# eminwux/kukeon

Hardware: AMD Instinct MI355X
Metric: agent_turns_per_sec (higher is better)
Workload: dtype bf16; 1 GPU; model=llama-3-8b, global_batch=64, seq_len=3584, parallelism=dp1, sessions_per_gpu_group=64, prompt_len=512, followup_len=256, decode_len=128

## Files before the change

### kukeon_amd/models/llama.py

```python
from __future__ import annotations

from dataclasses import dataclass
from typing import Optional

import torch
import torch.nn as nn
import torch.nn.functional as F

from kukeon_amd import ops
from kukeon_amd import parallel
from kukeon_amd.engine.config import ModelConfig


@dataclass
class AttnMeta:
    mode: str
    positions: torch.Tensor
    slot_mapping: torch.Tensor
    block_table: torch.Tensor
    seq_lens: torch.Tensor
    q_starts: Optional[torch.Tensor] = None
    qb_seq: Optional[torch.Tensor] = None
    qb_start: Optional[torch.Tensor] = None
    num_splits: int = 1
# ... 49 lines not shown
        import os
        weight_dtype = os.environ.get("KUKEON_WEIGHT_DTYPE") or "bf16"
    if weight_dtype not in WEIGHT_DTYPES:
        raise ValueError(f"weight_dtype must be one of {WEIGHT_DTYPES}, "
                         f"got {weight_dtype!r}")
    return weight_dtype


def _make_weight(shape, device, weight_dtype: str):
    w = _init_weight(shape, device)
    if weight_dtype == "fp8":
        return ops.quantize_weight(w.data)
    return w


class LlamaAttention(nn.Module):
    def __init__(self, cfg: ModelConfig, layer_idx: int, device,
                 weight_dtype: str = "bf16"):
        super().__init__()
        tp = parallel.tp_size()
        assert cfg.num_q_heads % tp == 0 and cfg.num_kv_heads % tp == 0, (
            "TP degree must divide q and kv head counts")
        self.layer_idx = layer_idx
        self.hq = cfg.num_q_heads // tp
        self.hk = cfg.num_kv_heads // tp
        self.d = cfg.head_dim
        self.scale = cfg.head_dim ** -0.5
        qkv_out = (self.hq + 2 * self.hk) * self.d
        self.qkv_w = _make_weight((qkv_out, cfg.hidden_size), device,
                                  weight_dtype)
        self.o_w = _make_weight((cfg.hidden_size, self.hq * self.d), device,
                                weight_dtype)

    def forward(self, x: torch.Tensor, cos_sin: torch.Tensor,
                kc: torch.Tensor, vc: torch.Tensor, meta: AttnMeta):
        qkv = ops.linear(x, self.qkv_w)
        ops.rope_kv_append(qkv, kc, vc, cos_sin, meta.positions,
                           meta.slot_mapping, self.hq, self.hk, self.d,
                           block_table=(meta.block_table
                                        if meta.mode == "decode" else None))
        out = torch.empty(x.shape[0], self.hq * self.d, dtype=x.dtype,
                          device=x.device)
        if meta.mode == "decode":
            ops.paged_attention(out, qkv, kc, vc, meta.block_table,
                                meta.seq_lens, 0, meta.num_splits, self.scale,
                                meta.tmp_out, meta.tmp_ml)
        else:
            ops.prefill_attention(out, qkv, kc, vc, meta.block_table,
                                  meta.seq_lens, meta.q_starts, meta.qb_seq,
                                  meta.qb_start, 0, self.scale)
        o = ops.linear(out, self.o_w)
        return parallel.tp_all_reduce(o)

    def forward_pre_o(self, x: torch.Tensor, cos_sin: torch.Tensor,
                      kc: torch.Tensor, vc: torch.Tensor, meta: AttnMeta):
        qkv = ops.linear(x, self.qkv_w)
        ops.rope_kv_append(qkv, kc, vc, cos_sin, meta.positions,
                           meta.slot_mapping, self.hq, self.hk, self.d,
                           block_table=(meta.block_table
                                        if meta.mode == "decode" else None))
        out = torch.empty(x.shape[0], self.hq * self.d, dtype=x.dtype,
                          device=x.device)
        if meta.mode == "decode":
            ops.paged_attention(out, qkv, kc, vc, meta.block_table,
                                meta.seq_lens, 0, meta.num_splits, self.scale,
                                meta.tmp_out, meta.tmp_ml)
        else:
            ops.prefill_attention(out, qkv, kc, vc, meta.block_table,
                                  meta.seq_lens, meta.q_starts, meta.qb_seq,
                                  meta.qb_start, 0, self.scale)
        return out


class LlamaMLP(nn.Module):
    def __init__(self, cfg: ModelConfig, device, weight_dtype: str = "bf16"):
        super().__init__()
        tp = parallel.tp_size()
        assert cfg.intermediate_size % tp == 0
        self.inter = cfg.intermediate_size // tp
        self.gate_up_w = _make_weight((2 * self.inter, cfg.hidden_size),
                                      device, weight_dtype)
        self.down_w = _make_weight((cfg.hidden_size, self.inter), device,
                                   weight_dtype)

    def forward(self, x: torch.Tensor) -> torch.Tensor:
        gu = ops.linear(x, self.gate_up_w)
        act = torch.empty(x.shape[0], self.inter, dtype=x.dtype,
                          device=x.device)
        ops.silu_mul(act, gu)
        return parallel.tp_all_reduce(ops.linear(act, self.down_w))


class LlamaLayer(nn.Module):
    def __init__(self, cfg: ModelConfig, layer_idx: int, device,
                 weight_dtype: str = "bf16"):
        super().__init__()
        self.input_norm = nn.Parameter(
            torch.ones(cfg.hidden_size, dtype=torch.bfloat16, device=device),
            requires_grad=False)
        self.post_norm = nn.Parameter(
            torch.ones(cfg.hidden_size, dtype=torch.bfloat16, device=device),
            requires_grad=False)
        self.attn = LlamaAttention(cfg, layer_idx, device, weight_dtype)
        self.mlp = LlamaMLP(cfg, device, weight_dtype)
# ... 148 lines not shown
```

### kukeon_amd/ops/__init__.py

```python
from __future__ import annotations

import torch

from . import reference

_C = None
_IMPORT_ERROR: Exception | None = None


def _load() -> None:
    global _C, _IMPORT_ERROR
    try:
        from kukeon_amd import _C as ext
    except Exception as e:
        _IMPORT_ERROR = e
    else:
        _C, _IMPORT_ERROR = ext, None


_load()


def native_available() -> bool:
    if _C is None:
# ... 17 lines not shown


def rmsnorm(out, input, weight, eps: float) -> None:
    _impl(input).rmsnorm(out, input, weight, eps)


def fused_add_rmsnorm(input, residual, weight, eps: float) -> None:
    _impl(input).fused_add_rmsnorm(input, residual, weight, eps)


def silu_mul(out, gate_up) -> None:
    _impl(gate_up).silu_mul(out, gate_up)


def rope_kv_append(qkv, k_cache, v_cache, cos_sin, positions, slot_mapping,
                   num_q_heads: int, num_kv_heads: int, head_dim: int,
                   block_table=None) -> None:
    if block_table is None:
        block_table = torch.empty(0, dtype=torch.int32, device=qkv.device)
    _impl(qkv).rope_kv_append(qkv, k_cache, v_cache, cos_sin, positions,
                              slot_mapping, num_q_heads, num_kv_heads,
                              head_dim, block_table)


def decode_advance(ids, pos, seq_lens, tokens, ring, counter) -> None:
    _impl(ids).decode_advance(ids, pos, seq_lens, tokens, ring, counter)


def paged_attention(out, q, k_cache, v_cache, block_table, seq_lens,
                    q_offset: int, num_splits: int, scale: float,
                    tmp_out, tmp_ml) -> None:
    _impl(q).paged_attention(out, q, k_cache, v_cache, block_table, seq_lens,
                             q_offset, num_splits, scale, tmp_out, tmp_ml)


def prefill_attention(out, q, k_cache, v_cache, block_table, seq_lens,
                      q_starts, qb_seq, qb_start, q_offset: int,
                      scale: float) -> None:
    _impl(q).prefill_attention(out, q, k_cache, v_cache, block_table,
                               seq_lens, q_starts, qb_seq, qb_start, q_offset,
                               scale)


def sample(tokens, logits, temps, top_k, top_p, seed, workspace) -> None:
    _impl(logits).sample(tokens, logits, temps, top_k, top_p, seed, workspace)


_SKINNY_WS = {}
_SKINNY_WS_RETIRED = []
_USE_SKINNY = __import__("os").environ.get("KUKEON_SKINNY_GEMM", "0")
_FUSE_SILU = __import__("os").environ.get("KUKEON_FUSE_SILU", "0") == "1"


def _skinny_wins(rows: int, N: int, K: int) -> bool:
    if _USE_SKINNY == "off":
        return False
    return N == K == 4096


def _skinny5_wins(rows: int, N: int, K: int) -> bool:
    if _USE_SKINNY == "off":
        return False
    return (N, K) in ((4096, 14336), (8192, 28672))


def _skinny_kind(x: torch.Tensor, w: torch.Tensor, fused: bool):
# ... 214 lines not shown
```

### kukeon_amd/ops/csrc/bindings.cpp

```cpp
#include <torch/extension.h>

namespace kukeon {
void rmsnorm(torch::Tensor out, torch::Tensor input, torch::Tensor weight,
             double eps);
void fused_add_rmsnorm(torch::Tensor input, torch::Tensor residual,
                       torch::Tensor weight, double eps);
void silu_mul(torch::Tensor out, torch::Tensor gate_up);
void rope_kv_append(torch::Tensor qkv, torch::Tensor k_cache,
                    torch::Tensor v_cache, torch::Tensor cos_sin,
                    torch::Tensor positions, torch::Tensor slot_mapping,
                    int64_t num_q_heads, int64_t num_kv_heads,
                    int64_t head_dim, torch::Tensor block_table);
void decode_advance(torch::Tensor ids, torch::Tensor pos,
                    torch::Tensor seq_lens, torch::Tensor tokens,
                    torch::Tensor ring, torch::Tensor counter);
void paged_attention(torch::Tensor out, torch::Tensor q, torch::Tensor k_cache,
                     torch::Tensor v_cache, torch::Tensor block_table,
                     torch::Tensor seq_lens, int64_t q_offset,
                     int64_t num_splits, double scale, torch::Tensor tmp_out,
                     torch::Tensor tmp_ml);
void prefill_attention(torch::Tensor out, torch::Tensor q,
                       torch::Tensor k_cache, torch::Tensor v_cache,
                       torch::Tensor block_table, torch::Tensor seq_lens,
                       torch::Tensor q_starts, torch::Tensor qb_seq,
                       torch::Tensor qb_start, int64_t q_offset, double scale);
void mfma_probe(torch::Tensor out, torch::Tensor a, torch::Tensor b);
void mfma_probe16(torch::Tensor out, torch::Tensor a, torch::Tensor b);
void mfma_probe16k(torch::Tensor out, torch::Tensor a, torch::Tensor b);
void skinny_gemm2(torch::Tensor out, torch::Tensor x, torch::Tensor w,
                  torch::Tensor ws);
void skinny_gemm5(torch::Tensor out, torch::Tensor x, torch::Tensor w,
                  torch::Tensor ws);
void skinny_gemm6(torch::Tensor out, torch::Tensor x, torch::Tensor w,
                  torch::Tensor ws);
void skinny_gemm5_silu_fused_norm(torch::Tensor normed, torch::Tensor gu,
                                  torch::Tensor w, torch::Tensor ws,
                                  torch::Tensor residual, torch::Tensor nw,
                                  double eps);
void skinny_gemm(torch::Tensor out, torch::Tensor x, torch::Tensor w,
                 torch::Tensor ws);
void glds_probe(torch::Tensor out, torch::Tensor src);
int64_t skinny_splitk(const std::string& kind, int64_t N, int64_t K);
void skinny_gemm5_fused_norm(torch::Tensor normed, torch::Tensor x,
                             torch::Tensor w, torch::Tensor ws,
                             torch::Tensor residual, torch::Tensor nw,
                             double eps);
void skinny_gemm_fused_norm(torch::Tensor normed, torch::Tensor x,
                            torch::Tensor w, torch::Tensor ws,
                            torch::Tensor residual, torch::Tensor nw,
                            double eps);
void skinny_gemm_w8(torch::Tensor out, torch::Tensor x, torch::Tensor q,
                    torch::Tensor scale, torch::Tensor ws);
void skinny_gemm_w8_fused_norm(torch::Tensor normed, torch::Tensor x,
// ... 2 lines not shown
                               torch::Tensor nw, double eps);
void quantize_fp8_rows(torch::Tensor q, torch::Tensor scale, torch::Tensor w);
void dequant_fp8_rows(torch::Tensor out, torch::Tensor q,
                      torch::Tensor scale);
void sample(torch::Tensor tokens, torch::Tensor logits, torch::Tensor temps,
            torch::Tensor top_k, torch::Tensor top_p, torch::Tensor seed,
            torch::Tensor workspace);
void moe_router_weights(torch::Tensor wdense, torch::Tensor logits,
                        long K);
void moe_dense_combine(torch::Tensor out, torch::Tensor y,
                       torch::Tensor wdense);
void moe_gather_tokens(torch::Tensor out, torch::Tensor input,
                       torch::Tensor row_map);
void moe_scatter_tokens(torch::Tensor out, torch::Tensor input,
                        torch::Tensor row_map, torch::Tensor weights,
                        int64_t top_k);
void moe_route_sort(torch::Tensor topk_w, torch::Tensor row_map,
                    torch::Tensor inv_map, torch::Tensor offsets,
                    torch::Tensor logits, long K);
void moe_grouped_gemm(torch::Tensor out, torch::Tensor a,
                      torch::Tensor a_rows, torch::Tensor w,
                      torch::Tensor offsets);
}

PYBIND11_MODULE(TORCH_EXTENSION_NAME, m) {
  m.def("rmsnorm", &kukeon::rmsnorm, "RMSNorm (bf16, gfx950)");
  m.def("fused_add_rmsnorm", &kukeon::fused_add_rmsnorm,
        "residual += input; input = rmsnorm(residual)");
  m.def("silu_mul", &kukeon::silu_mul, "out = silu(gate)*up from fused [T,2I]");
  m.def("rope_kv_append", &kukeon::rope_kv_append,
        "in-place NEOX RoPE on fused qkv + paged KV append");
  m.def("paged_attention", &kukeon::paged_attention,
        "decode paged attention (GQA, split-KV)");
  m.def("prefill_attention", &kukeon::prefill_attention,
        "varlen causal paged prefill attention (MFMA)");
  m.def("mfma_probe", &kukeon::mfma_probe,
        "32x32x16 bf16 MFMA fragment-layout probe");
  m.def("mfma_probe16", &kukeon::mfma_probe16,
        "16x16x32 bf16 MFMA fragment-layout probe");
  m.def("mfma_probe16k", &kukeon::mfma_probe16k,
        "16x16x16 (K=16) bf16 MFMA fragment-layout probe");
  m.def("skinny_gemm6", &kukeon::skinny_gemm6,
        "decode GEMM v6 (barrier-free register-x pipeline)");
  m.def("skinny_gemm5_silu_fused_norm",
        &kukeon::skinny_gemm5_silu_fused_norm,
        "silu(gate)*up + down GEMM + reduce + add + RMSNorm fused");
  m.def("skinny_gemm5", &kukeon::skinny_gemm5,
        "full-line W stream via wave-private LDS image (v5)");
  m.def("skinny_gemm2", &kukeon::skinny_gemm2,
        "G-walk hand-counted weight-streaming GEMM (v2)");
  m.def("skinny_gemm", &kukeon::skinny_gemm,
        "weight-streaming decode GEMM (M<=64)");
  m.def("skinny_splitk", &kukeon::skinny_splitk,
        "split-K factor the skinny launcher of `kind` (v1, v2, v5, v5_fused, "
        "v6, w8) uses for [N, K]; host-only",
        py::arg("kind"), py::arg("N"), py::arg("K"));
  m.def("glds_probe", &kukeon::glds_probe,
        "asm global_lds round-trip validator");
  m.def("skinny_gemm5_fused_norm", &kukeon::skinny_gemm5_fused_norm,
        "skinny5 + fused split-K reduce + residual add + RMSNorm");
  m.def("skinny_gemm_fused_norm", &kukeon::skinny_gemm_fused_norm,
        "skinny GEMM + split-K reduce + residual add + RMSNorm");
  m.def("skinny_gemm_w8", &kukeon::skinny_gemm_w8,
        "W8A16 decode GEMM: (x @ fp8(q)^T) * scale, M<=64");
  m.def("skinny_gemm_w8_fused_norm", &kukeon::skinny_gemm_w8_fused_norm,
        "W8A16 decode GEMM + split-K reduce + residual add + RMSNorm");
// ... 20 lines not shown
```

### kukeon_amd/ops/csrc/common.h

```cpp
#pragma once

#include <hip/hip_runtime.h>
#include <hip/hip_bf16.h>
#include <hip/hip_fp16.h>
#include <stdint.h>

#define WAVE 64

#define DEV_INLINE __device__ __forceinline__

DEV_INLINE float bf2f(__hip_bfloat16 x) { return __bfloat162float(x); }
DEV_INLINE __hip_bfloat16 f2bf(float x) { return __float2bfloat16(x); }

DEV_INLINE float us2f(unsigned short u) {
  unsigned int w = ((unsigned int)u) << 16;
  return __builtin_bit_cast(float, w);
}
DEV_INLINE unsigned short f2us(float f) {
  unsigned int w = __builtin_bit_cast(unsigned int, f);
  unsigned int lsb = (w >> 16) & 1u;
  w += 0x7fffu + lsb;
  return (unsigned short)(w >> 16);
}

struct bf16x8 {
  uint4 raw;
  DEV_INLINE unsigned short us(int i) const {
    const unsigned int* p = reinterpret_cast<const unsigned int*>(&raw);
    return (unsigned short)((p[i >> 1] >> ((i & 1) * 16)) & 0xffffu);
  }
  DEV_INLINE float f(int i) const { return us2f(us(i)); }
};

DEV_INLINE bf16x8 load_bf16x8(const void* p) {
  bf16x8 v;
  v.raw = *reinterpret_cast<const uint4*>(p);
  return v;
}

DEV_INLINE uint4 pack_bf16x8(const float* f) {
  uint4 r;
  unsigned int* p = reinterpret_cast<unsigned int*>(&r);
#pragma unroll
  for (int i = 0; i < 4; ++i) {
    p[i] = (unsigned int)f2us(f[2 * i]) | ((unsigned int)f2us(f[2 * i + 1]) << 16);
  }
  return r;
}

typedef __attribute__((__vector_size__(2 * sizeof(float)))) float f32x2_cvt_t;

DEV_INLINE unsigned int cvtpk_bf16(float lo, float hi) {
  __hip_bfloat162 h = __float22bfloat162_rn(float2{lo, hi});
  unsigned int r;
  __builtin_memcpy(&r, &h, 4);
  return r;
}

DEV_INLINE uint2 fp8x4_to_bf16x4(unsigned int w) {
  f32x2_cvt_t lo = __builtin_amdgcn_cvt_pk_f32_fp8(w, false);
  f32x2_cvt_t hi = __builtin_amdgcn_cvt_pk_f32_fp8(w, true);
  return uint2{cvtpk_bf16(lo[0], lo[1]), cvtpk_bf16(hi[0], hi[1])};
}

DEV_INLINE uint4 fp8x8_to_bf16x8(uint2 w) {
  const uint2 a = fp8x4_to_bf16x4(w.x);
  const uint2 b = fp8x4_to_bf16x4(w.y);
  return uint4{a.x, a.y, b.x, b.y};
}

DEV_INLINE uint2 pack_fp8x8(const float* f) {
  unsigned int w0 = __builtin_amdgcn_cvt_pk_fp8_f32(f[0], f[1], 0u, false);
  w0 = __builtin_amdgcn_cvt_pk_fp8_f32(f[2], f[3], w0, true);
  unsigned int w1 = __builtin_amdgcn_cvt_pk_fp8_f32(f[4], f[5], 0u, false);
  w1 = __builtin_amdgcn_cvt_pk_fp8_f32(f[6], f[7], w1, true);
  return uint2{w0, w1};
}

DEV_INLINE float wave_sum(float v) {
#pragma unroll
// ... 38 lines not shown
```

### kukeon_amd/ops/csrc/paged_attn.hip

```cpp
#include "attn_frag.h"
#include <torch/extension.h>
#include <c10/hip/HIPStream.h>

namespace kukeon {

template <bool FP8>
__global__ __launch_bounds__(256, FP8 ? 3 : 4) void paged_attn_kernel(
    float* __restrict__ tmp_out,
    float* __restrict__ tmp_ml,
    const unsigned short* __restrict__ q,
    const void* __restrict__ k_cache,
    const void* __restrict__ v_cache,
    const int* __restrict__ block_table,
    const int* __restrict__ seq_lens,
    long q_stride, int Hq, int Hk, int max_blocks, int S, float scale) {
  constexpr int D = 128;
  constexpr int BS = 16;
  const int b = blockIdx.x;
  const int hk = blockIdx.y;
  const int wid = threadIdx.x / WAVE;
  const int lane = threadIdx.x & (WAVE - 1);
  const int g4 = lane >> 4;
  const int rc = lane & 15;
  const int G = Hq / Hk;
  const int slot = blockIdx.z * 4 + wid;
  const int ctx = seq_lens[b];
  if (ctx <= 0 || slot >= S) return;

  __shared__ __align__(16) unsigned short vtbuf[4][2][D * BS];

  const int nblocks = (ctx + BS - 1) / BS;
  const int per_slot = (nblocks + S - 1) / S;
  const int blk_begin = slot * per_slot;
  const int blk_end = min(nblocks, blk_begin + per_slot);
  const int kv_hi = min(ctx, blk_end * BS);

  const int qh = min(rc, G - 1);
  unsigned int qf[4][4];
  {
    const unsigned short* qp =
        q + (long)b * q_stride + (long)(hk * G + qh) * D;
#pragma unroll
    for (int st = 0; st < 4; ++st) {
      const uint4 v = *reinterpret_cast<const uint4*>(qp + st * 32 + g4 * 8);
      qf[st][0] = v.x; qf[st][1] = v.y; qf[st][2] = v.z; qf[st][3] = v.w;
    }
  }

  float m = -INFINITY, l_acc = 0.f;
  f32x4_t oacc[8] = {{}, {}, {}, {}, {}, {}, {}, {}};

  const auto* kc = reinterpret_cast<const kv_elem_t<FP8>*>(k_cache);
  const auto* vc = reinterpret_cast<const kv_elem_t<FP8>*>(v_cache);

  uint4 kfr[4];
  auto kfetch = [&](int bi_f) {
    const long base =
        ((long)block_table[(long)b * max_blocks + bi_f] * Hk + hk) * BS * D;
    const long off = base + (long)rc * D + g4 * 8;
#pragma unroll
    for (int st = 0; st < 4; ++st)
      kfr[st] = load_kv8(kc + off + st * 32);
  };
  const int stg_d0 = rc * 8;
  uint4 vpre[2][2];
  auto vfetch = [&](int bi_f) {
    const long base =
        ((long)block_table[(long)b * max_blocks + bi_f] * Hk + hk) * BS * D;
#pragma unroll
    for (int pass = 0; pass < 2; ++pass) {
      const int kp = pass * 4 + g4;
      const long voff0 = base + (long)(2 * kp) * D + stg_d0;
      const long voff1 = base + (long)(2 * kp + 1) * D + stg_d0;
      vpre[pass][0] = load_kv8(vc + voff0);
      vpre[pass][1] = load_kv8(vc + voff1);
    }
  };
  auto vwrite = [&](unsigned short* vt, int kvbase) {
#pragma unroll
    for (int pass = 0; pass < 2; ++pass) {
      const int kp = pass * 4 + g4;
      uint4 r0 = vpre[pass][0];
      uint4 r1 = vpre[pass][1];
      if (kvbase + 2 * kp >= kv_hi) r0 = uint4{0, 0, 0, 0};
      if (kvbase + 2 * kp + 1 >= kv_hi) r1 = uint4{0, 0, 0, 0};
      const unsigned int* a0 = reinterpret_cast<const unsigned int*>(&r0);
      const unsigned int* a1 = reinterpret_cast<const unsigned int*>(&r1);
#pragma unroll
      for (int j = 0; j < 8; ++j) {
        const unsigned short e0 = (a0[j >> 1] >> ((j & 1) * 16)) & 0xffffu;
        const unsigned short e1 = (a1[j >> 1] >> ((j & 1) * 16)) & 0xffffu;
        const unsigned int packed = (unsigned)e0 | ((unsigned)e1 << 16);
        const int d = stg_d0 + j;
        const int byte = d * 32 + ((4 * kp) ^ ((d & 3) << 3));
        *reinterpret_cast<unsigned int*>(
            reinterpret_cast<char*>(vt) + byte) = packed;
      }
    }
  };

  if (blk_begin < blk_end) {
    kfetch(blk_begin);
    vfetch(blk_begin);
    vwrite(vtbuf[wid][blk_begin & 1], blk_begin * BS);
  }

  for (int bi = blk_begin; bi < blk_end; ++bi) {
    const int kvbase = bi * BS;
    const unsigned short* vt = vtbuf[wid][bi & 1];

    f32x4_t sacc = {};
#pragma unroll
    for (int st = 0; st < 4; ++st) {
      sacc = __builtin_amdgcn_mfma_f32_16x16x32_bf16(
          as_frag(kfr[st].x, kfr[st].y, kfr[st].z, kfr[st].w),
          as_frag(qf[st][0], qf[st][1], qf[st][2], qf[st][3]),
          sacc, 0, 0, 0);
    }
    if (bi + 1 < blk_end) kfetch(bi + 1);

    float sv[4];
    float tmax = -INFINITY;
#pragma unroll
    for (int r = 0; r < 4; ++r) {
      const bool valid = (kvbase + 4 * g4 + r) < kv_hi;
      sv[r] = valid ? sacc[r] * scale : -INFINITY;
      tmax = fmaxf(tmax, sv[r]);
    }
    tmax = fmaxf(tmax, __shfl_xor(tmax, 16, WAVE));
    tmax = fmaxf(tmax, __shfl_xor(tmax, 32, WAVE));
    const float mn = fmaxf(m, tmax);
    const float alpha = (m == -INFINITY) ? 0.f : __expf(m - mn);
    m = mn;
    float psum = 0.f;
#pragma unroll
    for (int r = 0; r < 4; ++r) {
      sv[r] = (sv[r] == -INFINITY) ? 0.f : __expf(sv[r] - mn);
      psum += sv[r];
    }
    psum += __shfl_xor(psum, 16, WAVE);
    psum += __shfl_xor(psum, 32, WAVE);
    l_acc = l_acc * alpha + psum;
#pragma unroll
    for (int dc = 0; dc < 8; ++dc)
#pragma unroll
      for (int r = 0; r < 4; ++r) oacc[dc][r] *= alpha;

    if (bi + 1 < blk_end) {
      vfetch(bi + 1);
      vwrite(vtbuf[wid][(bi + 1) & 1], (bi + 1) * BS);
    }

    const bf16x4_t pfrag = as_frag(cvtpk_bf16(sv[0], sv[1]),
                                   cvtpk_bf16(sv[2], sv[3]));
#pragma unroll
    for (int dc = 0; dc < 8; ++dc) {
      const int d = dc * 16 + rc;
      const int byte = d * 32 + ((8 * g4) ^ ((d & 3) << 3));
      const uint2 vf = *reinterpret_cast<const uint2*>(
          reinterpret_cast<const char*>(vt) + byte);
      oacc[dc] = __builtin_amdgcn_mfma_f32_16x16x16bf16_1k(
          as_frag(vf.x, vf.y), pfrag, oacc[dc], 0, 0, 0);
    }
  }

  if (rc >= G) return;
  const int head = hk * G + rc;
  float* top = tmp_out + (((long)b * Hq + head) * S + slot) * D;
#pragma unroll
  for (int dc = 0; dc < 8; ++dc) {
#pragma unroll
    for (int r = 0; r < 4; ++r) {
      top[dc * 16 + 4 * g4 + r] = oacc[dc][r];
    }
  }
  if (g4 == 0) {
    float* ml = tmp_ml + (((long)b * Hq + head) * S + slot) * 2;
    ml[0] = m;
    ml[1] = l_acc;
  }
}

template <int D>
__global__ void paged_attn_reduce_kernel(
    unsigned short* __restrict__ out, const float* __restrict__ tmp_out,
    const float* __restrict__ tmp_ml, const int* __restrict__ seq_lens,
    int Hq, int S) {
  const int b = blockIdx.x;
  const int h = blockIdx.y;
  const int d = threadIdx.x;
  if (seq_lens[b] <= 0) return;
  const float* ml = tmp_ml + (((long)b * Hq + h) * S) * 2;
  float M = -INFINITY;
  for (int s = 0; s < S; ++s) M = fmaxf(M, ml[s * 2]);
  float L = 0.f;
  for (int s = 0; s < S; ++s)
    L += (ml[s * 2] == -INFINITY ? 0.f : __expf(ml[s * 2] - M)) *
         ml[s * 2 + 1];
  const float* top = tmp_out + (((long)b * Hq + h) * S) * D;
  float acc = 0.f;
  for (int s = 0; s < S; ++s) {
    const float w = ml[s * 2] == -INFINITY ? 0.f : __expf(ml[s * 2] - M);
    acc += w * top[(long)s * D + d];
  }
  out[(long)b * Hq * D + (long)h * D + d] = f2us(L > 0.f ? acc / L : 0.f);
}

void paged_attention(torch::Tensor out, torch::Tensor q, torch::Tensor k_cache,
                     torch::Tensor v_cache, torch::Tensor block_table,
                     torch::Tensor seq_lens, int64_t q_offset,
                     int64_t num_splits, double scale, torch::Tensor tmp_out,
                     torch::Tensor tmp_ml) {
  const int B = q.size(0);
  if (B == 0) return;
  TORCH_CHECK(k_cache.dim() == 4 && k_cache.size(2) == 16 &&
                  k_cache.size(3) == 128,
              "kv caches must be [NB, Hk, 16, 128] (block size 16, "
              "head_dim 128)");
  TORCH_CHECK(v_cache.sizes() == k_cache.sizes() &&
                  v_cache.scalar_type() == k_cache.scalar_type() &&
                  k_cache.is_contiguous() && v_cache.is_contiguous(),
              "k_cache and v_cache must be contiguous and alike");
  const bool fp8 = k_cache.scalar_type() == torch::kUInt8;
  TORCH_CHECK(fp8 || k_cache.scalar_type() == torch::kBFloat16,
              "kv caches must be bf16 or uint8 (fp8 e4m3)");
  constexpr int D = 128;
  const int Hk = k_cache.size(1);
  TORCH_CHECK(out.dim() == 2 && out.size(0) == B && out.size(1) % D == 0 &&
                  out.scalar_type() == torch::kBFloat16 && out.is_contiguous(),
              "out must be contiguous bf16 [B, Hq*128]");
  const int Hq = out.size(1) / D;
  TORCH_CHECK(Hq >= Hk && Hq % Hk == 0 && Hq / Hk <= 16,
              "GQA group Hq/Hk must be an integer <= 16, got Hq=", Hq,
              " Hk=", Hk);
  TORCH_CHECK(q.scalar_type() == torch::kBFloat16 && q.dim() == 2 &&
                  q.stride(1) == 1,
              "q must be bf16 [B, >= Hq*128] with unit inner stride");
  TORCH_CHECK(q.stride(0) % 8 == 0 && q_offset % 8 == 0 && q_offset >= 0 &&
                  q_offset + (int64_t)Hq * D <= q.size(1),
              "q.stride(0) and q_offset must be multiples of 8 and the heads "
              "must fit in a q row, got stride ", q.stride(0), " offset ",
              q_offset);
  TORCH_CHECK(block_table.scalar_type() == torch::kInt32 &&
                  block_table.dim() == 2 && block_table.is_contiguous() &&
                  block_table.size(0) >= B,
              "block_table must be contiguous int32 [>= B, max_blocks]");
  TORCH_CHECK(seq_lens.scalar_type() == torch::kInt32 &&
                  seq_lens.is_contiguous() && seq_lens.numel() >= B,
              "seq_lens must be contiguous int32 [>= B]");
  TORCH_CHECK(num_splits >= 1, "num_splits must be >= 1");
  const int64_t slots = (int64_t)B * Hq * num_splits;
  TORCH_CHECK(tmp_out.scalar_type() == torch::kFloat32 &&
                  tmp_out.is_contiguous() && tmp_out.numel() >= slots * D,
              "tmp_out must be contiguous float32 with >= B*Hq*num_splits*128 "
              "elements, got ", tmp_out.numel(), " need ", slots * D);
  TORCH_CHECK(tmp_ml.scalar_type() == torch::kFloat32 &&
                  tmp_ml.is_contiguous() && tmp_ml.numel() >= slots * 2,
              "tmp_ml must be contiguous float32 with >= B*Hq*num_splits*2 "
              "elements, got ", tmp_ml.numel(), " need ", slots * 2);
  for (const auto& t : {out, k_cache, v_cache, block_table, seq_lens, tmp_out,
                        tmp_ml})
    TORCH_CHECK(t.device() == q.device() && t.is_cuda(),
                "all tensors must be on the same GPU");

  auto stream = c10::hip::getCurrentHIPStream().stream();
  const unsigned short* qp =
      reinterpret_cast<const unsigned short*>(q.data_ptr()) + q_offset;
  auto* launch = fp8 ? paged_attn_kernel<true> : paged_attn_kernel<false>;
  launch<<<dim3(B, Hk, (unsigned)((num_splits + 3) / 4)), 256, 0, stream>>>(
      tmp_out.data_ptr<float>(), tmp_ml.data_ptr<float>(), qp,
      k_cache.data_ptr(), v_cache.data_ptr(), block_table.data_ptr<int>(),
      seq_lens.data_ptr<int>(), q.stride(0), Hq, Hk,
      (int)block_table.size(1), (int)num_splits, (float)scale);
  HIP_CHECK_KERNEL();
  paged_attn_reduce_kernel<128><<<dim3(B, Hq), 128, 0, stream>>>(
      reinterpret_cast<unsigned short*>(out.data_ptr()),
      tmp_out.data_ptr<float>(), tmp_ml.data_ptr<float>(),
      seq_lens.data_ptr<int>(), Hq, (int)num_splits);
  HIP_CHECK_KERNEL();
}

}
```

### kukeon_amd/ops/csrc/rope_kv.hip

```cpp
#include "common.h"
#include <torch/extension.h>
#include <c10/hip/HIPStream.h>

namespace kukeon {

template <bool FP8>
__global__ void rope_kv_kernel(
    unsigned short* __restrict__ qkv,
    void* __restrict__ k_cache,
    void* __restrict__ v_cache,
    const float* __restrict__ cos_sin,
    const int* __restrict__ positions,
    const int* __restrict__ slot_mapping,
    const int* __restrict__ block_table,
    int max_blocks,
    int Hq, int Hk, int D, int BS) {
  const long t = blockIdx.x;
  const int yoff = blockIdx.y * blockDim.x + threadIdx.x;
  const int ystride = gridDim.y * blockDim.x;
  const int half = D / 2;
  const long row_stride = (long)(Hq + 2 * Hk) * D;
  unsigned short* row = qkv + t * row_stride;
  const int pos = positions[t];
  if (pos < 0) return;
  int slot;
  if (block_table != nullptr) {
    slot = block_table[t * (long)max_blocks + pos / BS] * BS + pos % BS;
  } else {
    slot = slot_mapping[t];
  }
  const float* cs = cos_sin + (long)pos * D;

  const int q_chunks = Hq * (D / 16);
  for (int c = yoff; c < q_chunks; c += ystride) {
    const int h = c / (D / 16);
    const int d0 = (c % (D / 16)) * 8;
    unsigned short* base = row + (long)h * D;
    bf16x8 x = load_bf16x8(base + d0);
    bf16x8 y = load_bf16x8(base + half + d0);
    float xo[8], yo[8];
#pragma unroll
    for (int j = 0; j < 8; ++j) {
      const float co = cs[d0 + j], si = cs[half + d0 + j];
      xo[j] = x.f(j) * co - y.f(j) * si;
      yo[j] = y.f(j) * co + x.f(j) * si;
    }
    *reinterpret_cast<uint4*>(base + d0) = pack_bf16x8(xo);
    *reinterpret_cast<uint4*>(base + half + d0) = pack_bf16x8(yo);
  }

  const long cache_tok_base =
      slot >= 0 ? ((long)(slot / BS) * Hk * BS + (long)(slot % BS)) * D : 0;
  const int k_chunks = Hk * (D / 16);
  for (int c = yoff; c < k_chunks; c += ystride) {
    const int h = c / (D / 16);
    const int d0 = (c % (D / 16)) * 8;
    unsigned short* base = row + (long)(Hq + h) * D;
    bf16x8 x = load_bf16x8(base + d0);
    bf16x8 y = load_bf16x8(base + half + d0);
    float xo[8], yo[8];
#pragma unroll
    for (int j = 0; j < 8; ++j) {
      const float co = cs[d0 + j], si = cs[half + d0 + j];
      xo[j] = x.f(j) * co - y.f(j) * si;
      yo[j] = y.f(j) * co + x.f(j) * si;
    }
    uint4 px = pack_bf16x8(xo), py = pack_bf16x8(yo);
    *reinterpret_cast<uint4*>(base + d0) = px;
    *reinterpret_cast<uint4*>(base + half + d0) = py;
    if (slot >= 0) {
      const long off = cache_tok_base + (long)h * BS * D;
      if (FP8) {
        unsigned char* kc = reinterpret_cast<unsigned char*>(k_cache) + off;
        *reinterpret_cast<uint2*>(kc + d0) = pack_fp8x8(xo);
        *reinterpret_cast<uint2*>(kc + half + d0) = pack_fp8x8(yo);
      } else {
        unsigned short* kc = reinterpret_cast<unsigned short*>(k_cache) + off;
        *reinterpret_cast<uint4*>(kc + d0) = px;
        *reinterpret_cast<uint4*>(kc + half + d0) = py;
      }
    }
  }

  if (slot >= 0) {
    const int v_chunks = Hk * (D / 8);
    for (int c = yoff; c < v_chunks; c += ystride) {
      const int h = c / (D / 8);
      const int d0 = (c % (D / 8)) * 8;
      const unsigned short* base = row + (long)(Hq + Hk + h) * D;
      const long off = cache_tok_base + (long)h * BS * D;
      if (FP8) {
        bf16x8 v = load_bf16x8(base + d0);
        float f[8];
#pragma unroll
        for (int j = 0; j < 8; ++j) f[j] = v.f(j);
        unsigned char* vc = reinterpret_cast<unsigned char*>(v_cache) + off;
        *reinterpret_cast<uint2*>(vc + d0) = pack_fp8x8(f);
      } else {
        unsigned short* vc = reinterpret_cast<unsigned short*>(v_cache) + off;
// ... 37 lines not shown
```

### kukeon_amd/ops/reference.py

```python
from __future__ import annotations

import torch


def rmsnorm(out: torch.Tensor, input: torch.Tensor, weight: torch.Tensor,
            eps: float) -> None:
    x = input.float()
    rs = torch.rsqrt(x.pow(2).mean(-1, keepdim=True) + eps)
    out.copy_((x * rs * weight.float()).to(out.dtype))


def fused_add_rmsnorm(input: torch.Tensor, residual: torch.Tensor,
                      weight: torch.Tensor, eps: float) -> None:
    r = (residual.float() + input.float())
    residual.copy_(r.to(residual.dtype))
    r = residual.float()
    rs = torch.rsqrt(r.pow(2).mean(-1, keepdim=True) + eps)
    input.copy_((r * rs * weight.float()).to(input.dtype))


def silu_mul(out: torch.Tensor, gate_up: torch.Tensor) -> None:
    I = out.shape[-1]
    g = gate_up[..., :I].float()
    u = gate_up[..., I:].float()
# ... 57 lines not shown
    nb = (ctx + BS - 1) // BS
    blocks = block_table[b, :nb].long()
    flat = cache[blocks]
    if flat.dtype == torch.uint8:
        flat = flat.view(torch.float8_e4m3fn).float()
    flat = flat.permute(0, 2, 1, 3).reshape(nb * BS, cache.shape[1], -1)
    return flat[:ctx]


def paged_attention(out: torch.Tensor, q: torch.Tensor, k_cache: torch.Tensor,
                    v_cache: torch.Tensor, block_table: torch.Tensor,
                    seq_lens: torch.Tensor, q_offset: int, num_splits: int,
                    scale: float, tmp_out=None, tmp_ml=None) -> None:
    B = q.shape[0]
    Hk, BS, D = k_cache.shape[1], k_cache.shape[2], k_cache.shape[3]
    Hq = out.shape[1] // D
    G = Hq // Hk
    qv = q.view(B, -1)[:, q_offset: q_offset + Hq * D].view(B, Hq, D).float()
    for b in range(B):
        ctx = int(seq_lens[b])
        if ctx <= 0:
            out.view(B, -1)[b] = 0
            continue
        k = _gather_kv(k_cache, block_table, ctx, b).float()
        v = _gather_kv(v_cache, block_table, ctx, b).float()
        for h in range(Hq):
            hk = h // G
            s = (k[:, hk] @ qv[b, h]) * scale
            p = torch.softmax(s, dim=-1)
            o = p @ v[:, hk]
            out.view(B, Hq, D)[b, h] = o.to(out.dtype)


def prefill_attention(out: torch.Tensor, q: torch.Tensor,
                      k_cache: torch.Tensor, v_cache: torch.Tensor,
                      block_table: torch.Tensor, seq_lens: torch.Tensor,
                      q_starts: torch.Tensor, qb_seq=None, qb_start=None,
                      q_offset: int = 0, scale: float = 1.0) -> None:
    Hk, BS, D = k_cache.shape[1], k_cache.shape[2], k_cache.shape[3]
    Hq = out.shape[1] // D
    G = Hq // Hk
    nseq = seq_lens.shape[0]
    for s in range(nseq):
        ctx = int(seq_lens[s])
        start = int(q_starts[s, 0])
        row = int(q_starts[s, 1])
        qlen = ctx - start
        if qlen <= 0:
            continue
        k = _gather_kv(k_cache, block_table, ctx, s).float()
        v = _gather_kv(v_cache, block_table, ctx, s).float()
        qs = q[row: row + qlen, q_offset: q_offset + Hq * D].view(
            qlen, Hq, D).float()
        pos = torch.arange(start, ctx)
        kvpos = torch.arange(ctx)
        mask = kvpos[None, :] <= pos[:, None]
        for h in range(Hq):
            hk = h // G
            sc = (qs[:, h] @ k[:, hk].T) * scale
            sc = sc.masked_fill(~mask, float("-inf"))
            p = torch.softmax(sc, dim=-1)
            o = p @ v[:, hk]
            out[row: row + qlen].view(qlen, Hq, D)[:, h] = o.to(out.dtype)
        pass


# ... 131 lines not shown
```

Before: 49.18 turns/s.

## Fold RoPE and KV append into decode attention and merge splits in-kernel

```diff
diff --git a/kukeon_amd/models/llama.py b/kukeon_amd/models/llama.py
--- a/kukeon_amd/models/llama.py
+++ b/kukeon_amd/models/llama.py
@@ -105,35 +105,23 @@
         self.o_w = _make_weight((cfg.hidden_size, self.hq * self.d), device,
                                 weight_dtype)
 
-    def forward(self, x: torch.Tensor, cos_sin: torch.Tensor,
+    def _attend(self, x: torch.Tensor, cos_sin: torch.Tensor,
                 kc: torch.Tensor, vc: torch.Tensor, meta: AttnMeta):
         qkv = ops.linear(x, self.qkv_w)
+        out = torch.empty(x.shape[0], self.hq * self.d, dtype=x.dtype,
+                          device=x.device)
+        if (meta.mode == "decode" and ops.DECODE_ATTN_FUSED
+                and kc.dtype != torch.uint8):
+            ops.paged_attention_rope(out, qkv, kc, vc, cos_sin,
+                                     meta.positions, meta.block_table,
+                                     meta.seq_lens, self.hq, self.hk,
+                                     meta.num_splits, self.scale,
+                                     meta.tmp_out, meta.tmp_ml)
+            return out
         ops.rope_kv_append(qkv, kc, vc, cos_sin, meta.positions,
                            meta.slot_mapping, self.hq, self.hk, self.d,
                            block_table=(meta.block_table
                                         if meta.mode == "decode" else None))
-        out = torch.empty(x.shape[0], self.hq * self.d, dtype=x.dtype,
-                          device=x.device)
-        if meta.mode == "decode":
-            ops.paged_attention(out, qkv, kc, vc, meta.block_table,
-                                meta.seq_lens, 0, meta.num_splits, self.scale,
-                                meta.tmp_out, meta.tmp_ml)
-        else:
-            ops.prefill_attention(out, qkv, kc, vc, meta.block_table,
-                                  meta.seq_lens, meta.q_starts, meta.qb_seq,
-                                  meta.qb_start, 0, self.scale)
-        o = ops.linear(out, self.o_w)
-        return parallel.tp_all_reduce(o)
-
-    def forward_pre_o(self, x: torch.Tensor, cos_sin: torch.Tensor,
-                      kc: torch.Tensor, vc: torch.Tensor, meta: AttnMeta):
-        qkv = ops.linear(x, self.qkv_w)
-        ops.rope_kv_append(qkv, kc, vc, cos_sin, meta.positions,
-                           meta.slot_mapping, self.hq, self.hk, self.d,
-                           block_table=(meta.block_table
-                                        if meta.mode == "decode" else None))
-        out = torch.empty(x.shape[0], self.hq * self.d, dtype=x.dtype,
-                          device=x.device)
         if meta.mode == "decode":
             ops.paged_attention(out, qkv, kc, vc, meta.block_table,
                                 meta.seq_lens, 0, meta.num_splits, self.scale,
@@ -143,6 +131,16 @@
                                   meta.seq_lens, meta.q_starts, meta.qb_seq,
                                   meta.qb_start, 0, self.scale)
         return out
+
+    def forward(self, x: torch.Tensor, cos_sin: torch.Tensor,
+                kc: torch.Tensor, vc: torch.Tensor, meta: AttnMeta):
+        out = self._attend(x, cos_sin, kc, vc, meta)
+        o = ops.linear(out, self.o_w)
+        return parallel.tp_all_reduce(o)
+
+    def forward_pre_o(self, x: torch.Tensor, cos_sin: torch.Tensor,
+                      kc: torch.Tensor, vc: torch.Tensor, meta: AttnMeta):
+        return self._attend(x, cos_sin, kc, vc, meta)
 
 
 class LlamaMLP(nn.Module):
diff --git a/kukeon_amd/ops/__init__.py b/kukeon_amd/ops/__init__.py
--- a/kukeon_amd/ops/__init__.py
+++ b/kukeon_amd/ops/__init__.py
@@ -73,6 +73,20 @@
                     tmp_out, tmp_ml) -> None:
     _impl(q).paged_attention(out, q, k_cache, v_cache, block_table, seq_lens,
                              q_offset, num_splits, scale, tmp_out, tmp_ml)
+
+
+DECODE_ATTN_FUSED = __import__("os").environ.get(
+    "KUKEON_DECODE_ATTN_FUSED", "1") != "0"
+
+
+def paged_attention_rope(out, qkv, k_cache, v_cache, cos_sin, positions,
+                         block_table, seq_lens, num_q_heads: int,
+                         num_kv_heads: int, num_splits: int, scale: float,
+                         tmp_out, tmp_ml) -> None:
+    _impl(qkv).paged_attention_rope(out, qkv, k_cache, v_cache, cos_sin,
+                                    positions, block_table, seq_lens,
+                                    num_q_heads, num_kv_heads, num_splits,
+                                    scale, tmp_out, tmp_ml)
 
 
 def prefill_attention(out, q, k_cache, v_cache, block_table, seq_lens,
diff --git a/kukeon_amd/ops/csrc/bindings.cpp b/kukeon_amd/ops/csrc/bindings.cpp
--- a/kukeon_amd/ops/csrc/bindings.cpp
+++ b/kukeon_amd/ops/csrc/bindings.cpp
@@ -19,6 +19,13 @@
                      torch::Tensor seq_lens, int64_t q_offset,
                      int64_t num_splits, double scale, torch::Tensor tmp_out,
                      torch::Tensor tmp_ml);
+void paged_attention_rope(torch::Tensor out, torch::Tensor qkv,
+                          torch::Tensor k_cache, torch::Tensor v_cache,
+                          torch::Tensor cos_sin, torch::Tensor positions,
+                          torch::Tensor block_table, torch::Tensor seq_lens,
+                          int64_t num_q_heads, int64_t num_kv_heads,
+                          int64_t num_splits, double scale,
+                          torch::Tensor tmp_out, torch::Tensor tmp_ml);
 void prefill_attention(torch::Tensor out, torch::Tensor q,
                        torch::Tensor k_cache, torch::Tensor v_cache,
                        torch::Tensor block_table, torch::Tensor seq_lens,
@@ -87,6 +94,8 @@
         "in-place NEOX RoPE on fused qkv + paged KV append");
   m.def("paged_attention", &kukeon::paged_attention,
         "decode paged attention (GQA, split-KV)");
+  m.def("paged_attention_rope", &kukeon::paged_attention_rope,
+        "decode paged attention with RoPE + KV append folded in");
   m.def("prefill_attention", &kukeon::prefill_attention,
         "varlen causal paged prefill attention (MFMA)");
   m.def("mfma_probe", &kukeon::mfma_probe,
diff --git a/kukeon_amd/ops/csrc/common.h b/kukeon_amd/ops/csrc/common.h
--- a/kukeon_amd/ops/csrc/common.h
+++ b/kukeon_amd/ops/csrc/common.h
@@ -46,6 +46,17 @@
     p[i] = (unsigned int)f2us(f[2 * i]) | ((unsigned int)f2us(f[2 * i + 1]) << 16);
   }
   return r;
+}
+
+DEV_INLINE void rope_rotate8(const bf16x8& x, const bf16x8& y,
+                             const float* co, const float* si, float* xo,
+                             float* yo) {
+#pragma unroll
+  for (int j = 0; j < 8; ++j) {
+    const float c = co[j], s = si[j];
+    xo[j] = __builtin_fmaf(x.f(j), c, -(y.f(j) * s));
+    yo[j] = __builtin_fmaf(x.f(j), s, y.f(j) * c);
+  }
 }
 
 typedef __attribute__((__vector_size__(2 * sizeof(float)))) float f32x2_cvt_t;
diff --git a/kukeon_amd/ops/csrc/paged_attn.hip b/kukeon_amd/ops/csrc/paged_attn.hip
--- a/kukeon_amd/ops/csrc/paged_attn.hip
+++ b/kukeon_amd/ops/csrc/paged_attn.hip
@@ -4,16 +4,26 @@
 
 namespace kukeon {
 
-template <bool FP8>
-__global__ __launch_bounds__(256, FP8 ? 3 : 4) void paged_attn_kernel(
+DEV_INLINE float merge_weight(float m_s, float M) {
+  return m_s == -INFINITY ? 0.f : __expf(m_s - M);
+}
+
+constexpr int kWaveLds = 2 * 128 * 16 * 2;
+
+template <bool FP8, bool ROPE>
+__global__ __launch_bounds__(512, 4) void paged_attn_kernel(
+    unsigned short* __restrict__ out,
     float* __restrict__ tmp_out,
     float* __restrict__ tmp_ml,
     const unsigned short* __restrict__ q,
-    const void* __restrict__ k_cache,
-    const void* __restrict__ v_cache,
+    void* k_cache,
+    void* v_cache,
+    const float* __restrict__ cos_sin,
+    const int* __restrict__ positions,
     const int* __restrict__ block_table,
     const int* __restrict__ seq_lens,
-    long q_stride, int Hq, int Hk, int max_blocks, int S, float scale) {
+    long q_stride, int Hq, int Hk, int max_blocks, int S, int merge,
+    float scale) {
   constexpr int D = 128;
   constexpr int BS = 16;
   const int b = blockIdx.x;
@@ -23,14 +33,56 @@
   const int g4 = lane >> 4;
   const int rc = lane & 15;
   const int G = Hq / Hk;
-  const int slot = blockIdx.z * 4 + wid;
+  const int slot = blockIdx.z * (blockDim.x / WAVE) + wid;
   const int ctx = seq_lens[b];
-  if (ctx <= 0 || slot >= S) return;
-
-  __shared__ __align__(16) unsigned short vtbuf[4][2][D * BS];
-
-  const int nblocks = (ctx + BS - 1) / BS;
+
+  const int nblocks = ctx > 0 ? (ctx + BS - 1) / BS : 0;
   const int per_slot = (nblocks + S - 1) / S;
+
+  const int pos = ROPE ? positions[b] : -1;
+  if (ROPE && pos >= 0) {
+    const int pblk = pos / BS;
+    const int owner = pblk < nblocks ? pblk / per_slot : 0;
+    if (slot == owner && pblk < max_blocks && lane < 16) {
+      const unsigned short* krow =
+          q + (long)b * q_stride + (long)(Hq + hk) * D;
+      const unsigned short* vrow = krow + (long)Hk * D;
+      const long dst =
+          (((long)block_table[(long)b * max_blocks + pblk] * Hk + hk) * BS +
+           pos % BS) * D;
+      auto* kdst = reinterpret_cast<kv_elem_t<FP8>*>(k_cache) + dst;
+      auto* vdst = reinterpret_cast<kv_elem_t<FP8>*>(v_cache) + dst;
+      if (lane < 8) {
+        const int d0 = lane * 8;
+        const float* cs = cos_sin + (long)pos * D;
+        float xo[8], yo[8];
+        rope_rotate8(load_bf16x8(krow + d0), load_bf16x8(krow + D / 2 + d0),
+                     cs + d0, cs + D / 2 + d0, xo, yo);
+        if constexpr (FP8) {
+          *reinterpret_cast<uint2*>(kdst + d0) = pack_fp8x8(xo);
+          *reinterpret_cast<uint2*>(kdst + D / 2 + d0) = pack_fp8x8(yo);
+        } else {
+          *reinterpret_cast<uint4*>(kdst + d0) = pack_bf16x8(xo);
+          *reinterpret_cast<uint4*>(kdst + D / 2 + d0) = pack_bf16x8(yo);
+        }
+      }
+      const bf16x8 v = load_bf16x8(vrow + lane * 8);
+      if constexpr (FP8) {
+        float f[8];
+#pragma unroll
+        for (int j = 0; j < 8; ++j) f[j] = v.f(j);
+        *reinterpret_cast<uint2*>(vdst + lane * 8) = pack_fp8x8(f);
+      } else {
+        *reinterpret_cast<uint4*>(vdst + lane * 8) = v.raw;
+      }
+    }
+    __threadfence_block();
+  }
+  if (ctx <= 0 || (!merge && slot >= S)) return;
+
+  extern __shared__ __align__(16) unsigned short vtbuf_all[];
+  unsigned short* const vtbuf0 = vtbuf_all + wid * (2 * D * BS);
+
   const int blk_begin = slot * per_slot;
   const int blk_end = min(nblocks, blk_begin + per_slot);
   const int kv_hi = min(ctx, blk_end * BS);
@@ -40,9 +92,24 @@
   {
     const unsigned short* qp =
         q + (long)b * q_stride + (long)(hk * G + qh) * D;
+    bf16x8 qv[4];
+#pragma unroll
+    for (int st = 0; st < 4; ++st)
+      qv[st] = load_bf16x8(qp + st * 32 + g4 * 8);
+    if (ROPE && pos >= 0) {
+      const float* cs = cos_sin + (long)pos * D;
+#pragma unroll
+      for (int st = 0; st < 2; ++st) {
+        const int d0 = st * 32 + g4 * 8;
+        float xo[8], yo[8];
+        rope_rotate8(qv[st], qv[st + 2], cs + d0, cs + D / 2 + d0, xo, yo);
+        qv[st].raw = pack_bf16x8(xo);
+        qv[st + 2].raw = pack_bf16x8(yo);
+      }
+    }
 #pragma unroll
     for (int st = 0; st < 4; ++st) {
-      const uint4 v = *reinterpret_cast<const uint4*>(qp + st * 32 + g4 * 8);
+      const uint4 v = qv[st].raw;
       qf[st][0] = v.x; qf[st][1] = v.y; qf[st][2] = v.z; qf[st][3] = v.w;
     }
   }
@@ -102,12 +169,12 @@
   if (blk_begin < blk_end) {
     kfetch(blk_begin);
     vfetch(blk_begin);
-    vwrite(vtbuf[wid][blk_begin & 1], blk_begin * BS);
+    vwrite(vtbuf0 + (blk_begin & 1) * (D * BS), blk_begin * BS);
   }
 
   for (int bi = blk_begin; bi < blk_end; ++bi) {
     const int kvbase = bi * BS;
-    const unsigned short* vt = vtbuf[wid][bi & 1];
+    const unsigned short* vt = vtbuf0 + (bi & 1) * (D * BS);
 
     f32x4_t sacc = {};
 #pragma unroll
@@ -148,7 +215,7 @@
 
     if (bi + 1 < blk_end) {
       vfetch(bi + 1);
-      vwrite(vtbuf[wid][(bi + 1) & 1], (bi + 1) * BS);
+      vwrite(vtbuf0 + ((bi + 1) & 1) * (D * BS), (bi + 1) * BS);
     }
 
     const bf16x4_t pfrag = as_frag(cvtpk_bf16(sv[0], sv[1]),
@@ -164,20 +231,77 @@
     }
   }
 
-  if (rc >= G) return;
-  const int head = hk * G + rc;
-  float* top = tmp_out + (((long)b * Hq + head) * S + slot) * D;
+  if (!merge) {
+    if (rc >= G) return;
+    const int head = hk * G + rc;
+    float* top = tmp_out + (((long)b * Hq + head) * S + slot) * D;
+#pragma unroll
+    for (int dc = 0; dc < 8; ++dc) {
+#pragma unroll
+      for (int r = 0; r < 4; ++r) {
+        top[dc * 16 + 4 * g4 + r] = oacc[dc][r];
+      }
+    }
+    if (g4 == 0) {
+      float* ml = tmp_ml + (((long)b * Hq + head) * S + slot) * 2;
+      ml[0] = m;
+      ml[1] = l_acc;
+    }
+    return;
+  }
+
+  char* const lds = reinterpret_cast<char*>(vtbuf_all);
+  __syncthreads();
+  if (rc < G && slot < S) {
+    if (wid > 0) {
+      float4* op = reinterpret_cast<float4*>(lds + wid * kWaveLds + rc * 512);
+#pragma unroll
+      for (int dc = 0; dc < 8; ++dc)
+        op[(dc * 4 + g4) ^ rc] =
+            float4{oacc[dc][0], oacc[dc][1], oacc[dc][2], oacc[dc][3]};
+    }
+    if (g4 == 0)
+      reinterpret_cast<float2*>(lds)[wid * 16 + rc] = float2{m, l_acc};
+  }
+  __syncthreads();
+  if (wid != 0 || rc >= G) return;
+  const float2* ml = reinterpret_cast<const float2*>(lds) + rc;
+  float M = -INFINITY;
+  for (int s = 0; s < S; ++s) M = fmaxf(M, ml[s * 16].x);
+  float L = 0.f;
+  for (int s = 0; s < S; ++s)
+    L = __builtin_fmaf(merge_weight(ml[s * 16].x, M), ml[s * 16].y, L);
+  f32x4_t acc[8];
+  {
+    const float w = merge_weight(ml[0].x, M);
+#pragma unroll
+    for (int dc = 0; dc < 8; ++dc)
+#pragma unroll
+      for (int r = 0; r < 4; ++r)
+        acc[dc][r] = __builtin_fmaf(w, oacc[dc][r], 0.f);
+  }
+  for (int s = 1; s < S; ++s) {
+    const float w = merge_weight(ml[s * 16].x, M);
+    const float4* op =
+        reinterpret_cast<const float4*>(lds + s * kWaveLds + rc * 512);
+#pragma unroll
+    for (int dc = 0; dc < 8; ++dc) {
+      const float4 o = op[(dc * 4 + g4) ^ rc];
+      acc[dc][0] = __builtin_fmaf(w, o.x, acc[dc][0]);
+      acc[dc][1] = __builtin_fmaf(w, o.y, acc[dc][1]);
+      acc[dc][2] = __builtin_fmaf(w, o.z, acc[dc][2]);
+      acc[dc][3] = __builtin_fmaf(w, o.w, acc[dc][3]);
+    }
+  }
+  unsigned short* orow = out + (long)b * Hq * D + (long)(hk * G + rc) * D;
 #pragma unroll
   for (int dc = 0; dc < 8; ++dc) {
-#pragma unroll
-    for (int r = 0; r < 4; ++r) {
-      top[dc * 16 + 4 * g4 + r] = oacc[dc][r];
-    }
-  }
-  if (g4 == 0) {
-    float* ml = tmp_ml + (((long)b * Hq + head) * S + slot) * 2;
-    ml[0] = m;
-    ml[1] = l_acc;
+    unsigned short e[4];
+#pragma unroll
+    for (int r = 0; r < 4; ++r) e[r] = f2us(L > 0.f ? acc[dc][r] / L : 0.f);
+    *reinterpret_cast<uint2*>(orow + dc * 16 + 4 * g4) =
+        uint2{(unsigned)e[0] | ((unsigned)e[1] << 16),
+              (unsigned)e[2] | ((unsigned)e[3] << 16)};
   }
 }
 
@@ -195,22 +319,24 @@
   for (int s = 0; s < S; ++s) M = fmaxf(M, ml[s * 2]);
   float L = 0.f;
   for (int s = 0; s < S; ++s)
-    L += (ml[s * 2] == -INFINITY ? 0.f : __expf(ml[s * 2] - M)) *
-         ml[s * 2 + 1];
+    L = __builtin_fmaf(merge_weight(ml[s * 2], M), ml[s * 2 + 1], L);
   const float* top = tmp_out + (((long)b * Hq + h) * S) * D;
   float acc = 0.f;
   for (int s = 0; s < S; ++s) {
-    const float w = ml[s * 2] == -INFINITY ? 0.f : __expf(ml[s * 2] - M);
-    acc += w * top[(long)s * D + d];
+    const float w = merge_weight(ml[s * 2], M);
+    acc = __builtin_fmaf(w, top[(long)s * D + d], acc);
   }
   out[(long)b * Hq * D + (long)h * D + d] = f2us(L > 0.f ? acc / L : 0.f);
 }
 
-void paged_attention(torch::Tensor out, torch::Tensor q, torch::Tensor k_cache,
-                     torch::Tensor v_cache, torch::Tensor block_table,
-                     torch::Tensor seq_lens, int64_t q_offset,
-                     int64_t num_splits, double scale, torch::Tensor tmp_out,
-                     torch::Tensor tmp_ml) {
+static void decode_attention(torch::Tensor out, torch::Tensor q,
+                             torch::Tensor k_cache, torch::Tensor v_cache,
+                             const torch::Tensor* cos_sin,
+                             const torch::Tensor* positions,
+                             torch::Tensor block_table, torch::Tensor seq_lens,
+                             int64_t q_offset, int64_t num_splits,
+                             double scale, torch::Tensor tmp_out,
+                             torch::Tensor tmp_ml) {
   const int B = q.size(0);
   if (B == 0) return;
   TORCH_CHECK(k_cache.dim() == 4 && k_cache.size(2) == 16 &&
@@ -263,21 +389,76 @@
     TORCH_CHECK(t.device() == q.device() && t.is_cuda(),
                 "all tensors must be on the same GPU");
 
+  const bool rope = cos_sin != nullptr;
+  const float* csp = nullptr;
+  const int* posp = nullptr;
+  if (rope) {
+    TORCH_CHECK(q_offset == 0 && q.is_contiguous() &&
+                    q.size(1) == (int64_t)(Hq + 2 * Hk) * D,
+                "qkv must be contiguous bf16 [B, (Hq+2*Hk)*128]");
+    TORCH_CHECK(cos_sin->scalar_type() == torch::kFloat32 &&
+                    cos_sin->dim() == 2 && cos_sin->size(1) == D &&
+                    cos_sin->is_contiguous(),
+                "cos_sin must be contiguous float32 [max_pos, 128]");
+    TORCH_CHECK(positions->scalar_type() == torch::kInt32 &&
+                    positions->is_contiguous() && positions->numel() >= B,
+                "positions must be contiguous int32 [>= B]");
+    for (const auto* t : {cos_sin, positions})
+      TORCH_CHECK(t->device() == q.device(),
+                  "all tensors must be on the same GPU");
+    csp = cos_sin->data_ptr<float>();
+    posp = positions->data_ptr<int>();
+  }
+
+  const int S = (int)num_splits;
+  const bool merge = S <= 8;
+  const int waves = merge && S > 4 ? 8 : 4;
   auto stream = c10::hip::getCurrentHIPStream().stream();
   const unsigned short* qp =
       reinterpret_cast<const unsigned short*>(q.data_ptr()) + q_offset;
-  auto* launch = fp8 ? paged_attn_kernel<true> : paged_attn_kernel<false>;
-  launch<<<dim3(B, Hk, (unsigned)((num_splits + 3) / 4)), 256, 0, stream>>>(
+  auto* launch = fp8 ? (rope ? paged_attn_kernel<true, true>
+                             : paged_attn_kernel<true, false>)
+                     : (rope ? paged_attn_kernel<false, true>
+                             : paged_attn_kernel<false, false>);
+  launch<<<dim3(B, Hk, (unsigned)((S + waves - 1) / waves)), waves * WAVE,
+           waves * kWaveLds, stream>>>(
+      reinterpret_cast<unsigned short*>(out.data_ptr()),
       tmp_out.data_ptr<float>(), tmp_ml.data_ptr<float>(), qp,
-      k_cache.data_ptr(), v_cache.data_ptr(), block_table.data_ptr<int>(),
-      seq_lens.data_ptr<int>(), q.stride(0), Hq, Hk,
-      (int)block_table.size(1), (int)num_splits, (float)scale);
+      k_cache.data_ptr(), v_cache.data_ptr(), csp, posp,
+      block_table.data_ptr<int>(), seq_lens.data_ptr<int>(), q.stride(0), Hq,
+      Hk, (int)block_table.size(1), S, (int)merge, (float)scale);
   HIP_CHECK_KERNEL();
+  if (merge) return;
   paged_attn_reduce_kernel<128><<<dim3(B, Hq), 128, 0, stream>>>(
       reinterpret_cast<unsigned short*>(out.data_ptr()),
       tmp_out.data_ptr<float>(), tmp_ml.data_ptr<float>(),
-      seq_lens.data_ptr<int>(), Hq, (int)num_splits);
+      seq_lens.data_ptr<int>(), Hq, S);
   HIP_CHECK_KERNEL();
 }
 
-}
+void paged_attention(torch::Tensor out, torch::Tensor q, torch::Tensor k_cache,
+                     torch::Tensor v_cache, torch::Tensor block_table,
+                     torch::Tensor seq_lens, int64_t q_offset,
+                     int64_t num_splits, double scale, torch::Tensor tmp_out,
+                     torch::Tensor tmp_ml) {
+  decode_attention(out, q, k_cache, v_cache, nullptr, nullptr, block_table,
+                   seq_lens, q_offset, num_splits, scale, tmp_out, tmp_ml);
+}
+
+void paged_attention_rope(torch::Tensor out, torch::Tensor qkv,
+                          torch::Tensor k_cache, torch::Tensor v_cache,
+                          torch::Tensor cos_sin, torch::Tensor positions,
+                          torch::Tensor block_table, torch::Tensor seq_lens,
+                          int64_t num_q_heads, int64_t num_kv_heads,
+                          int64_t num_splits, double scale,
+                          torch::Tensor tmp_out, torch::Tensor tmp_ml) {
+  TORCH_CHECK(out.dim() == 2 && out.size(1) == num_q_heads * 128 &&
+                  k_cache.dim() == 4 && k_cache.size(1) == num_kv_heads,
+              "out must be [B, num_q_heads*128] and the caches "
+              "[NB, num_kv_heads, 16, 128]");
+  decode_attention(out, qkv, k_cache, v_cache, &cos_sin, &positions,
+                   block_table, seq_lens, 0, num_splits, scale, tmp_out,
+                   tmp_ml);
+}
+
+}
diff --git a/kukeon_amd/ops/csrc/rope_kv.hip b/kukeon_amd/ops/csrc/rope_kv.hip
--- a/kukeon_amd/ops/csrc/rope_kv.hip
+++ b/kukeon_amd/ops/csrc/rope_kv.hip
@@ -39,12 +39,7 @@
     bf16x8 x = load_bf16x8(base + d0);
     bf16x8 y = load_bf16x8(base + half + d0);
     float xo[8], yo[8];
-#pragma unroll
-    for (int j = 0; j < 8; ++j) {
-      const float co = cs[d0 + j], si = cs[half + d0 + j];
-      xo[j] = x.f(j) * co - y.f(j) * si;
-      yo[j] = y.f(j) * co + x.f(j) * si;
-    }
+    rope_rotate8(x, y, cs + d0, cs + half + d0, xo, yo);
     *reinterpret_cast<uint4*>(base + d0) = pack_bf16x8(xo);
     *reinterpret_cast<uint4*>(base + half + d0) = pack_bf16x8(yo);
   }
@@ -59,12 +54,7 @@
     bf16x8 x = load_bf16x8(base + d0);
     bf16x8 y = load_bf16x8(base + half + d0);
     float xo[8], yo[8];
-#pragma unroll
-    for (int j = 0; j < 8; ++j) {
-      const float co = cs[d0 + j], si = cs[half + d0 + j];
-      xo[j] = x.f(j) * co - y.f(j) * si;
-      yo[j] = y.f(j) * co + x.f(j) * si;
-    }
+    rope_rotate8(x, y, cs + d0, cs + half + d0, xo, yo);
     uint4 px = pack_bf16x8(xo), py = pack_bf16x8(yo);
     *reinterpret_cast<uint4*>(base + d0) = px;
     *reinterpret_cast<uint4*>(base + half + d0) = py;
diff --git a/kukeon_amd/ops/reference.py b/kukeon_amd/ops/reference.py
--- a/kukeon_amd/ops/reference.py
+++ b/kukeon_amd/ops/reference.py
@@ -113,6 +113,21 @@
             out.view(B, Hq, D)[b, h] = o.to(out.dtype)
 
 
+def paged_attention_rope(out: torch.Tensor, qkv: torch.Tensor,
+                         k_cache: torch.Tensor, v_cache: torch.Tensor,
+                         cos_sin: torch.Tensor, positions: torch.Tensor,
+                         block_table: torch.Tensor, seq_lens: torch.Tensor,
+                         num_q_heads: int, num_kv_heads: int,
+                         num_splits: int, scale: float, tmp_out=None,
+                         tmp_ml=None) -> None:
+    rot = qkv.clone()
+    rope_kv_append(rot, k_cache, v_cache, cos_sin, positions, None,
+                   num_q_heads, num_kv_heads, k_cache.shape[3],
+                   block_table=block_table)
+    paged_attention(out, rot, k_cache, v_cache, block_table, seq_lens, 0,
+                    num_splits, scale, tmp_out, tmp_ml)
+
+
 def prefill_attention(out: torch.Tensor, q: torch.Tensor,
                       k_cache: torch.Tensor, v_cache: torch.Tensor,
                       block_table: torch.Tensor, seq_lens: torch.Tensor,
```

New measurement: 50.34 turns/s (median of 6 runs). +2.4%, better.
